# Penguin77jp/RaytracingMin

Measured on AMD Instinct MI355X. Metric: Msamples/s (W*H*spp/s), Cornell box 1080p@1024spp, higher is better.
Workload: dtype f64; 1 GPU; cornellBoxSetting.json rows 0:1080 of 1920x1080 1024spp (SS 4 x S 64), L1 repaired, max_bounces 8, seed 0x5EED, host-libm sin/cos (RTM_MODE_HOST_TRIG), interleaved 8-row bands over 1 GPU(s) + one gather; sample_split_waves_per_tile=8, collective=none (one rank, frame stays in HBM)

## Files before the change

include/rtm_debug.h:

```cpp
#ifndef RTM_DEBUG_H
#define RTM_DEBUG_H

#include "rtm.h"

#ifdef __cplusplus
extern "C" {
#endif

int rtm_debug_math_probe(int op, const double* a, const double* b, size_t n, double* out);
int rtm_debug_trig_table(int entries, double* out);
int rtm_debug_selfcheck(int kind, unsigned long long* mismatches);
int rtm_debug_wf_nearest(int kind, const rtm_sphere* spheres, size_t n, const double* org, const double* dir,
                         size_t n_rays, int32_t* out_id, double* out_t);
int rtm_debug_fp64_peak(int waves_per_simd, double min_ms, double* tflops, double* kernel_ms);
int rtm_debug_grid_nearest(const rtm_sphere* spheres, size_t n, const double* org, const double* dir, size_t n_rays,
                           int32_t* out_id, double* out_t, uint32_t* out_tests, uint32_t* out_steps, uint64_t* info);
int rtm_debug_grid_build(const rtm_sphere* spheres, size_t n, uint64_t* info, double* pads, uint32_t* ranges, size_t ranges_cap,
                         uint32_t* items, size_t items_cap, int32_t* big, size_t big_cap);
int rtm_debug_scene_grid(const rtm_scene* scene, uint64_t* info, uint32_t* ranges, size_t ranges_cap, uint32_t* items,
                         size_t items_cap, int32_t* big, size_t big_cap, uint64_t extra[2]);
int rtm_debug_scene_facts(const rtm_sphere* spheres, size_t n, uint64_t facts[2]);
int rtm_debug_zero_term_facts(const rtm_sphere* spheres, size_t n, uint64_t facts[2]);
int rtm_debug_axis_rows(const rtm_sphere* spheres, size_t n, double* rows);
int rtm_debug_wall_pairs(const rtm_sphere* spheres, size_t n, uint64_t facts[2]);
int rtm_debug_component_bench(int which, const rtm_sphere* spheres, size_t n, int reps, int blocks, int lds_pad,
                              double* cycles_per_rep);
int rtm_debug_denoise_variance_kernel(int form, const rtm_denoise_var_params* params, int32_t width, int32_t height, int device,
                                      const rtm_aov_buffers* guide_dev, void* work_dev, float* variance_out_dev, void* stream);
int rtm_debug_matte_rank(int32_t super_samples, int32_t layers, int device, const int32_t* ids_dev, size_t n_pixels,
                         int32_t* id_out_dev, float* coverage_out_dev, float* alpha_out_dev, void* stream);

#ifdef __cplusplus
}
#endif
#endif
```

raytracingmin_amd/_lib.py:

```python
import ctypes as C
import os

_HERE = os.path.dirname(os.path.abspath(__file__))
LIB_PATH = os.environ.get("RTM_LIB_OVERRIDE") or os.path.join(_HERE, "librtm_hip.so")

RTM_OK = 0
MODE_LITERAL, MODE_REPAIRED = 0, 1
MODE_HOST_TRIG = 0x100
MODE_COUNT_TESTS = 0x200
MODE_SURFACE_SAMPLE = 0x400
MODES = {"literal": MODE_LITERAL, "repaired": MODE_REPAIRED, 0: 0, 1: 1}


class RtmError(RuntimeError):
    def __init__(self, status, what, detail=""):
        self.status = status
        super().__init__(f"{what}: {detail}" if detail else what)


class rtm_camera(C.Structure):
    _fields_ = [("origin", C.c_double * 3), ("target", C.c_double * 3), ("up", C.c_double * 3),
                ("fov", C.c_float), ("_pad", C.c_float)]


# ... 186 lines not shown
    "rtm_read_pfm": (C.c_int, [C.c_char_p, _P(C.c_int), _P(C.c_int), _P(C.c_int), C.c_void_p, C.c_size_t]),
}
DEBUG_SIGNATURES = {
    "rtm_debug_math_probe": (C.c_int, [C.c_int, C.c_void_p, C.c_void_p, C.c_size_t, C.c_void_p]),
    "rtm_debug_selfcheck": (C.c_int, [C.c_int, C.POINTER(C.c_uint64)]),
    "rtm_debug_trig_table": (C.c_int, [C.c_int, C.c_void_p]),
    "rtm_debug_fp64_peak": (C.c_int, [C.c_int, C.c_double, C.POINTER(C.c_double), C.POINTER(C.c_double)]),
    "rtm_debug_wf_nearest": (C.c_int, [C.c_int, C.c_void_p, C.c_size_t, C.c_void_p, C.c_void_p, C.c_size_t,
                                       C.c_void_p, C.c_void_p]),
    "rtm_debug_grid_nearest": (C.c_int, [C.c_void_p, C.c_size_t, C.c_void_p, C.c_void_p, C.c_size_t, C.c_void_p, C.c_void_p,
                                         C.c_void_p, C.c_void_p, C.c_void_p]),
    "rtm_debug_scene_facts": (C.c_int, [C.c_void_p, C.c_size_t, C.c_void_p]),
    "rtm_debug_zero_term_facts": (C.c_int, [C.c_void_p, C.c_size_t, C.c_void_p]),
    "rtm_debug_axis_rows": (C.c_int, [C.c_void_p, C.c_size_t, C.c_void_p]),
    "rtm_debug_wall_pairs": (C.c_int, [C.c_void_p, C.c_size_t, C.c_void_p]),
    "rtm_debug_grid_build": (C.c_int, [C.c_void_p, C.c_size_t, C.c_void_p, C.c_void_p, C.c_void_p, C.c_size_t, C.c_void_p,
                                       C.c_size_t, C.c_void_p, C.c_size_t]),
    "rtm_debug_scene_grid": (C.c_int, [C.c_void_p, C.c_void_p, C.c_void_p, C.c_size_t, C.c_void_p, C.c_size_t, C.c_void_p, C.c_size_t,
                                       C.c_void_p]),
    "rtm_debug_denoise_variance_kernel": (C.c_int, [C.c_int, _P(rtm_denoise_var_params), C.c_int32, C.c_int32, C.c_int,
                                                    _P(rtm_aov_buffers), C.c_void_p, C.c_void_p, C.c_void_p]),
    "rtm_debug_matte_rank": (C.c_int, [C.c_int32, C.c_int32, C.c_int, C.c_void_p, C.c_size_t, C.c_void_p, C.c_void_p, C.c_void_p,
                                       C.c_void_p]),
    "rtm_debug_component_bench": (C.c_int, [C.c_int, C.c_void_p, C.c_size_t, C.c_int, C.c_int, C.c_int,
                                            C.POINTER(C.c_double)]),
}
ABI_VERSION = 5

_lib = None

# ... 33 lines not shown
```

raytracingmin_amd/csrc/rtm_api.cpp:

```cpp
#include <exception>

#include "../../include/rtm_debug.h"
#include "rtm_internal.h"

#define RTM_GUARD(call)                                  \
    try {                                                \
        return (call);                                   \
    } catch (const std::exception& e) {                  \
        rtm::set_last_error(e.what());                   \
        return RTM_ERR_INVALID_ARGUMENT;                 \
    } catch (...) {                                      \
        rtm::set_last_error("unknown exception");        \
        return RTM_ERR_INVALID_ARGUMENT;                 \
    }

extern "C" {

int rtm_abi_version(void) { return RTM_ABI_VERSION; }

const char* rtm_strerror(int status) {
    switch (status) {
        case RTM_OK: return "ok";
        case RTM_ERR_INVALID_ARGUMENT: return "invalid argument";
        case RTM_ERR_INVALID_SCENE: return "invalid scene";
// ... 183 lines not shown
                           int32_t* out_id, double* out_t, uint32_t* out_tests, uint32_t* out_steps, uint64_t* info) {
    RTM_GUARD(rtm::grid_nearest_probe(sp, n, org, dir, n_rays, out_id, out_t, out_tests, out_steps, info))
}
int rtm_debug_grid_build(const rtm_sphere* sp, size_t n, uint64_t* info, double* pads, uint32_t* ranges, size_t ranges_cap,
                         uint32_t* items, size_t items_cap, int32_t* big, size_t big_cap) {
    RTM_GUARD(rtm::grid_build_host(sp, n, info, pads, ranges, ranges_cap, items, items_cap, big, big_cap))
}
int rtm_debug_scene_grid(const rtm_scene* scene, uint64_t* info, uint32_t* ranges, size_t ranges_cap, uint32_t* items,
                         size_t items_cap, int32_t* big, size_t big_cap, uint64_t extra[2]) {
    RTM_GUARD(rtm::scene_grid_probe(scene, info, ranges, ranges_cap, items, items_cap, big, big_cap, extra))
}
int rtm_debug_scene_facts(const rtm_sphere* sp, size_t n, uint64_t facts[2]) { RTM_GUARD(rtm::scene_facts_host(sp, n, facts)) }
int rtm_debug_zero_term_facts(const rtm_sphere* sp, size_t n, uint64_t facts[2]) { RTM_GUARD(rtm::zero_term_facts_host(sp, n, facts)) }
int rtm_debug_axis_rows(const rtm_sphere* sp, size_t n, double* rows) { RTM_GUARD(rtm::axis_rows_host(sp, n, rows)) }
int rtm_debug_wall_pairs(const rtm_sphere* sp, size_t n, uint64_t facts[2]) { RTM_GUARD(rtm::wall_pairs_host(sp, n, facts)) }
int rtm_debug_fp64_peak(int waves_per_simd, double min_ms, double* tflops, double* kernel_ms) {
    RTM_GUARD(rtm::fp64_peak(waves_per_simd, min_ms, tflops, kernel_ms))
}

int rtm_scene_load_json(const char* path, int literal_loader, rtm_settings* settings,
                        rtm_sphere* spheres, size_t capacity, size_t* n_spheres) {
    RTM_GUARD(rtm::scene_load_json(path, literal_loader, settings, spheres, capacity, n_spheres))
}
int rtm_scene_parse_json(const char* text, size_t len, int literal_loader, rtm_settings* settings,
                         rtm_sphere* spheres, size_t capacity, size_t* n_spheres) {
    RTM_GUARD(rtm::scene_parse_json(text, len, literal_loader, settings, spheres, capacity, n_spheres))
}
int rtm_scene_save_sample_json(const char* path) { RTM_GUARD(rtm::scene_save_sample_json(path)) }
int rtm_scene_make_stress(uint64_t seed, size_t n, rtm_settings* settings, rtm_sphere* spheres) {
    RTM_GUARD(rtm::scene_make_stress(seed, n, settings, spheres))
// ... 35 lines not shown
```

raytracingmin_amd/csrc/rtm_device.h:

```cpp
#pragma once
#include <hip/hip_runtime.h>
#include <stdint.h>

#ifndef RTM_NS
#define RTM_NS rtm
#endif
#ifndef RTM_TOL
#define RTM_TOL 0
#endif

namespace RTM_NS {

struct D3 {
    double x, y, z;
};

__device__ __forceinline__ D3 d3(double x, double y, double z) { return D3{x, y, z}; }
__device__ __forceinline__ D3 operator+(D3 a, D3 b) { return D3{a.x + b.x, a.y + b.y, a.z + b.z}; }
__device__ __forceinline__ D3 operator-(D3 a, D3 b) { return D3{a.x - b.x, a.y - b.y, a.z - b.z}; }
__device__ __forceinline__ D3 operator*(D3 a, D3 b) { return D3{a.x * b.x, a.y * b.y, a.z * b.z}; }
__device__ __forceinline__ D3 operator*(D3 a, double s) { return D3{a.x * s, a.y * s, a.z * s}; }
__device__ __forceinline__ D3 operator/(D3 a, double s) { return D3{a.x / s, a.y / s, a.z / s}; }

__device__ __forceinline__ D3 fold_step(const D3 c, const D3 L, const D3 e) {
// ... 182 lines not shown
    const double cosv = c1 + __builtin_fma(t * t, p, c3);
    double s = __builtin_fma(t, k[10], k[11]);
    s = __builtin_fma(t, s, k[12]);
    s = __builtin_fma(t, s, k[13]);
    s = __builtin_fma(t, s, k[14]);
    const double v = hi * t;
    const double sinv = __builtin_fma(v, __builtin_fma(t, s, k[15]), hi);
    const LaneMask odd = lane_mask((q & 1) != 0);
    const int flip = (q & 2) ? (int)0x80000000 : 0;
    const double so = sel_f64(odd, cosv, sinv);
    const double co = sel_f64(odd, -sinv, cosv);
    sn = __hiloint2double(__double2hiint(so) ^ flip, __double2loint(so));
    cs = __hiloint2double(__double2hiint(co) ^ flip, __double2loint(co));
}
constexpr int kTrigTabEntries = 16384;
struct TrigTabWord {
    double s, c;
    int fi;
};
__device__ __forceinline__ TrigTabWord sincos_turn24_tab_load(const double2* __restrict__ tab, const uint32_t m) {
    const uint32_t t = m + 512u;
    unsigned off = (t >> 6) & ((unsigned)(kTrigTabEntries - 1) * (unsigned)sizeof(double2));
    asm volatile("" : "+v"(off));
    const double2 e = *reinterpret_cast<const double2*>(reinterpret_cast<const char*>(tab) + off);
    return TrigTabWord{e.x, e.y, (int)(t & 1023u) - 512};
}
__device__ __forceinline__ void sincos_tab_point_apply(const double ws, const double wc, const double r, double& sn, double& cs) {
    const double t = r * r;
    const double cr = __builtin_fma(t, __builtin_fma(t, 1.0 / 24.0, -0.5), 1.0);
    const double sr = __builtin_fma(r * t, -1.0 / 6.0, r);
// ... 66 lines not shown
```

raytracingmin_amd/csrc/rtm_internal.h:

```cpp
#pragma once
#include <stddef.h>
#include <stdint.h>

#include <string>

#include "../../include/rtm.h"

namespace rtm {

void set_last_error(const std::string& s);
const char* last_error();

int device_count(int* count);
int num_variants();
int output_rows(const rtm_options* opt);
int release_scratch(int device);
int stream_release(int device, void* stream);
int wf_nearest_probe(int kind, const rtm_sphere* sp, size_t n, const double* org, const double* dir, size_t n_rays,
                     int32_t* out_id, double* out_t);
const char* variant_name(int v);
int scene_create(const rtm_sphere* sp, size_t n, int on_device, int device, rtm_scene** out);
int scene_create_device(const rtm_sphere* sp_dev, size_t n, int device, void* stream, rtm_scene** out);
int scene_create_objects(const rtm_object* objs, size_t n, int device, rtm_scene** out);
int intersect_objects_batch(const rtm_object* objs, const double* org, const double* dir, size_t n, int mode,
// ... 66 lines not shown
int selfcheck(int kind, unsigned long long* mismatches);
int grid_nearest_probe(const rtm_sphere* sp, size_t n, const double* org, const double* dir, size_t n_rays, int32_t* out_id,
                       double* out_t, uint32_t* out_tests, uint32_t* out_steps, uint64_t* info);
int scene_facts_host(const rtm_sphere* sp, size_t n, uint64_t* facts);
int zero_term_facts_host(const rtm_sphere* sp, size_t n, uint64_t* facts);
int axis_rows_host(const rtm_sphere* sp, size_t n, double* rows);
int wall_pairs_host(const rtm_sphere* sp, size_t n, uint64_t* facts);
int grid_build_host(const rtm_sphere* sp, size_t n, uint64_t* info, double* pads, uint32_t* ranges, size_t ranges_cap,
                    uint32_t* items, size_t items_cap, int32_t* big, size_t big_cap);
int scene_grid_probe(const rtm_scene* sc, uint64_t* info, uint32_t* ranges, size_t ranges_cap, uint32_t* items, size_t items_cap,
                     int32_t* big, size_t big_cap, uint64_t* extra);
int fp64_peak(int waves_per_simd, double min_ms, double* tflops, double* kernel_ms);
int math_probe(int op, const double* a, const double* b, size_t n, double* out);
int launch_tol(const void* render_params, size_t params_bytes, unsigned grid, size_t lds_pad, void* stream);
int tol_math_probe(int op, const double* a_dev, const double* b_dev, size_t n, double* out_dev);
int trig_table_host(int entries, double* out);
void release_trig_tab(int device);

int scene_parse_json(const char* text, size_t len, int literal_loader, rtm_settings* st,
                     rtm_sphere* spheres, size_t capacity, size_t* n_spheres);
int scene_parse_json_objects(const char* text, size_t len, int literal_loader, rtm_settings* st,
                             rtm_object* objects, size_t capacity, size_t* n_objects);
int scene_load_json_objects(const char* path, int literal_loader, rtm_settings* st, rtm_object* objects,
                            size_t capacity, size_t* n_objects);
int scene_load_json(const char* path, int literal_loader, rtm_settings* st, rtm_sphere* spheres,
                    size_t capacity, size_t* n_spheres);
int scene_save_sample_json(const char* path);
int scene_make_stress(uint64_t seed, size_t n, rtm_settings* st, rtm_sphere* spheres);
int quantise(const double* image, size_t n_values, uint8_t* out);
int write_bmp(const char* filename, int w, int h, int comp, const void* data);
// ... 6 lines not shown
```

raytracingmin_amd/csrc/rtm_kernels.hip:

```cpp
#include <hip/hip_runtime.h>

#include <cfloat>
#include <cmath>
#include <cstdio>
#include <cstdlib>
#include <cstring>
#include <algorithm>
#include <atomic>
#include <thread>
#include <map>
#include <memory>
#include <mutex>
#include <shared_mutex>
#include <tuple>
#include <string>
#include <type_traits>
#include <vector>

#include "../../include/rtm.h"
#include "rtm_device.h"
#include "rtm_host.h"
#include "rtm_path.h"

#include "rtm_render_kernel.h"
// ... 1132 lines not shown
constexpr int deep_lds_levels() { return sizeof(RecT) == 1 ? 64 : 32; }
static bool needs_pool(const RenderParams& P) { return !(P.max_bounces >= 0 && P.max_bounces < 16); }

static size_t debug_lds_pad() {
    static const size_t pad = [] {
        const char* e = std::getenv("RTM_DEBUG_LDS_PAD");
        return e ? (size_t)std::strtoul(e, nullptr, 10) : (size_t)0;
    }();
    return pad;
}

template <class M, unsigned F, typename RecT, int LDS_D, int WPE>
static bool launch_exact_n(const RenderParams& P, unsigned grid, hipStream_t stream) {
    const size_t pad = debug_lds_pad();
    unsigned unit_tab;
    render_lds_bytes<F, RecT, LDS_D>(P.scene.n, pad, &unit_tab);
#define RTM_AXIS_CASE(k, sig)                                                                           \
    if (P.scene.n == k && P.scene.axis_pat == sig && P.mode == RTM_MODE_REPAIRED && unit_tab == 1u) {   \
        launch_tiles<M, F, axis_unroll(k, sig), RecT, LDS_D, WPE>(P, grid, pad, stream);                \
        return true;                                                                                    \
    }
    RTM_AXIS_SIGNATURES(RTM_AXIS_CASE)
#undef RTM_AXIS_CASE
    if constexpr ((F & kPack8) != 0) {
        switch (P.scene.n) {
#define RTM_EXACT_N(k)                                                             \
    case k:                                                                        \
        launch_tiles<M, F, -100 - k, RecT, LDS_D, WPE>(P, grid, pad, stream);      \
        return true;
            RTM_EXACT_N(1) RTM_EXACT_N(2) RTM_EXACT_N(3) RTM_EXACT_N(4) RTM_EXACT_N(5) RTM_EXACT_N(6) RTM_EXACT_N(7)
#undef RTM_EXACT_N
// ... 1617 lines not shown
```

raytracingmin_amd/csrc/rtm_kernels_tol.hip:

```cpp
#define RTM_NS rtm_tol
#define RTM_TOL 1
#include <hip/hip_runtime.h>

#include <cmath>
#include <cstdlib>
#include <cstring>
#include <map>
#include <mutex>
#include <vector>

#include "rtm_internal.h"
#include "rtm_render_kernel.h"

namespace rtm_tol {

static bool compact_launch(const RenderParams& P) {
    const double cam = std::sqrt(P.cam_org.x * P.cam_org.x + P.cam_org.y * P.cam_org.y + P.cam_org.z * P.cam_org.z);
    return (P.scene.fold_flags & kSceneCompact) != 0u && cam <= kCompactExtent;
}
static bool expanded_form_launch(const RenderParams& P) {
    const unsigned e = (P.scene.fold_flags >> kSceneAxisReachShift) & kSceneAxisReachMask;
    const double cam = std::sqrt(P.cam_org.x * P.cam_org.x + P.cam_org.y * P.cam_org.y + P.cam_org.z * P.cam_org.z);
    return e != 0u && cam <= std::ldexp(1.0, (int)e - 128);
}

constexpr unsigned kTolCapped = kLdsTab | kPark | kPack8 | kDefer | kSteal;
constexpr unsigned kTolAny = kLdsTab | kPark | kDefer | kPackL;
constexpr int kTolWavesPerSimd = 4;

template <unsigned F>
static void launch_n(const RenderParams& P, unsigned grid, size_t lds_pad, hipStream_t stream) {
    constexpr int LDS_D = (F & kPackL) != 0 ? 0 : 16;
    unsigned unit_tab;
    render_lds_bytes<F, uint8_t, LDS_D>(P.scene.n, lds_pad, &unit_tab);
    const bool axis = P.mode == RTM_MODE_REPAIRED && unit_tab == 1u && compact_launch(P) && expanded_form_launch(P);
    const unsigned shared_k = (P.scene.fold_flags >> kSceneSharedKShift) & kSceneSharedKMask;
    constexpr bool kPairsShape = (F & (kPackL | kSplit)) != (kPackL | kSplit);
    const unsigned pairs = kPairsShape && (P.scene.fold_flags & kSceneWallPairs) != 0u ? kAxisPairsBit : 0u;
#define RTM_AXIS_CASE(k, sig)                                                                                    \
    if (P.scene.n == k && P.scene.axis_pat == ((sig) & 0xFFFFu) && ((shared_k << kAxisSharedKShift) | pairs) == ((sig) & ~0xFFFFu) && axis) { \
        launch_tiles<MathFast, F, axis_unroll(k, sig), uint8_t, LDS_D, kTolWavesPerSimd>(P, grid, lds_pad, stream); \
        return;                                                                                                  \
    }
    if constexpr (kPairsShape) {
        RTM_AXIS_CASE(7, kAxisSigCornell7Pairs)
    }
    RTM_AXIS_CASE(7, kAxisSigCornell7Walls)
#undef RTM_AXIS_CASE
#define RTM_AXIS_CASE(k, sig)                                                                                    \
// ... 122 lines not shown
namespace rtm {

int trig_table_host(int entries, double* out) {
    if (!out || entries < 1 || entries > (1 << 20)) return RTM_ERR_INVALID_ARGUMENT;
    const long double step = 6.283185307179586476925286766559L / (long double)entries;
    for (int i = 0; i < entries; ++i) {
        const long double a = (long double)i * step;
        out[2 * i] = (double)sinl(a);
        out[2 * i + 1] = (double)cosl(a);
    }
    return RTM_OK;
}

namespace {
std::mutex g_trig_tab_mu;
std::map<int, double2*> g_trig_tab;
}

static int ensure_trig_tab(const double2** out) {
    int device = 0;
    if (hipGetDevice(&device) != hipSuccess) return RTM_ERR_HIP;
    std::lock_guard<std::mutex> lock(g_trig_tab_mu);
    const auto it = g_trig_tab.find(device);
    if (it != g_trig_tab.end()) {
        *out = it->second;
        return RTM_OK;
    }
    constexpr size_t kBytes = (size_t)rtm_tol::kTrigTabEntries * sizeof(double2);
    std::vector<double> host(2 * (size_t)rtm_tol::kTrigTabEntries);
    const int rc = trig_table_host(rtm_tol::kTrigTabEntries, host.data());
    if (rc != RTM_OK) return rc;
    void* dev = nullptr;
    if (hipMalloc(&dev, kBytes) != hipSuccess) {
        (void)hipGetLastError();
        return RTM_ERR_HIP;
    }
    if (hipMemcpy(dev, host.data(), kBytes, hipMemcpyHostToDevice) != hipSuccess || hipStreamSynchronize(nullptr) != hipSuccess) {
        (void)hipGetLastError();
        (void)hipFree(dev);
        return RTM_ERR_HIP;
    }
    g_trig_tab[device] = static_cast<double2*>(dev);
    *out = static_cast<const double2*>(dev);
    return RTM_OK;
}

void release_trig_tab(int device) {
    std::lock_guard<std::mutex> lock(g_trig_tab_mu);
    for (auto it = g_trig_tab.begin(); it != g_trig_tab.end();) {
        if (device < 0 || it->first == device) {
            (void)hipSetDevice(it->first);
            (void)hipDeviceSynchronize();
            (void)hipFree(it->second);
            it = g_trig_tab.erase(it);
        } else {
            ++it;
        }
    }
}

int tol_math_probe(int op, const double* a_dev, const double* b_dev, size_t n, double* out_dev) {
    const double2* tab = nullptr;
    if (op == 42 || op == 43 || op == 46 || op == 47) {
        if (ensure_trig_tab(&tab) != RTM_OK) {
            set_last_error("tolerance row: the sin / cos table could not be allocated on the device");
            return RTM_ERR_HIP;
        }
    }
    rtm_tol::tol_math_probe_kernel<<<(unsigned)((n + 255) / 256), 256>>>(op, a_dev, b_dev, n, out_dev, tab);
    return hipGetLastError() == hipSuccess ? RTM_OK : RTM_ERR_HIP;
}

int launch_tol(const void* params, size_t params_bytes, unsigned grid, size_t lds_pad, void* stream_v) {
    rtm_tol::RenderParams P;
    if (params_bytes != sizeof P) {
        set_last_error("tolerance row: RenderParams layout mismatch between the two translation units");
        return RTM_ERR_INVALID_ARGUMENT;
    }
    std::memcpy(&P, params, sizeof P);
    P.scene.trig_fix = nullptr;
    const double2* trig_tab = nullptr;
    if (ensure_trig_tab(&trig_tab) != RTM_OK) {
        set_last_error("tolerance row: the sin / cos table could not be allocated on the device");
        return RTM_ERR_HIP;
    }
    P.trig_tab = trig_tab;
    hipStream_t stream = (hipStream_t)stream_v;
    const bool any_depth = P.max_bounces < 0 || P.max_bounces > 8;
    if ((!any_depth && P.steal_ws == nullptr) || P.scene.n < 1 || P.scene.n > 24 || P.scene.plane != nullptr ||
        P.sample_end >= 65536u) {
        set_last_error("variant 18 (fp64 tolerance row) serves all-sphere scenes of 1..24 spheres with fewer than 65 536 samples per pixel");
        return RTM_ERR_UNSUPPORTED;
    }
    if (P.prim_masks == nullptr) {
        set_last_error("tolerance row: no primary-ray mask buffer");
        return RTM_ERR_INVALID_ARGUMENT;
    }
    const unsigned n_tiles_all = P.split > 1 ? P.split_first + P.n_tiles : grid;
    static const bool no_masks = [] {
        const char* e = std::getenv("RTM_DEBUG_TOL_PRIMFIX");
        return e && e[0] == '0';
// ... 18 lines not shown
```

raytracingmin_amd/csrc/rtm_path.h:

```cpp
#pragma once
#include <cfloat>
#include <type_traits>

#include "../../include/rtm.h"
#include "rtm_device.h"

namespace RTM_NS {


__device__ __forceinline__ double seq_rcp(const double y) {
    double r = __builtin_amdgcn_rcp(y);
    double e = __builtin_fma(-y, r, 1.0);
#if RTM_TOL
    return __builtin_fma(r, __builtin_fma(e, e, e), r);
#else
    r = __builtin_fma(r, e, r);
    e = __builtin_fma(-y, r, 1.0);
    return __builtin_fma(r, e, r);
#endif
}
__device__ __forceinline__ double seq_quot(const double x, const double y, const double r) {
#if RTM_TOL
    (void)y;
    return x * r;
// ... 545 lines not shown
        const double* g = lgeom + id * 4;
        return D3{g[0], g[1], g[2]};
    }
    __device__ __forceinline__ double kd(int id) const { return lmat[id * 8 + 6]; }
    __device__ __forceinline__ double kd24(int id) const { return lmat[id * 8 + 7]; }
    __device__ __forceinline__ D3 emission(int id) const {
        const double* m = lmat + id * 8;
        return D3{m[3], m[4], m[5]};
    }
    __device__ __forceinline__ D3 color_kd(int id) const {
        const double* m = lmat + id * 8;
        return D3{m[0], m[1], m[2]};
    }
};

struct SceneLdsObjects {
    SceneView v;
    const double* lgeom;
    const double* lmat;
    const double* lnrm;
    static constexpr bool kHasNormTable = false;
    static constexpr bool kPlanes = true;
    static constexpr bool kNeverPlanes = false;
    __device__ __forceinline__ int n() const { return v.n; }
    __device__ __forceinline__ double4 geom_uniform(int i) const { return load_geom_uniform(v.geom, i); }
    __device__ __forceinline__ D3 center(int id) const {
        const double* g = lgeom + id * 4;
        return D3{g[0], g[1], g[2]};
    }
    __device__ __forceinline__ bool is_plane(int id) const { return __double2hiint(lgeom[id * 4 + 3]) < 0; }
// ... 204 lines not shown
        b = py * dir.y - A.Pxz;
        D4 = b * b - (py * py + A.Qxz) + g.w;
    } else if (pat == 3u) {
        const double pz = g.z - org.z;
        b = pz * dir.z - A.Pxy;
        D4 = b * b - (A.Qxy + pz * pz) + g.w;
    } else {
        const D3 p_o = d3(g.x - org.x, g.y - org.y, g.z - org.z);
        b = dot(p_o, dir);
        D4 = b * b - dot(p_o, p_o) + g.w;
    }
}
__device__ __forceinline__ double pair_signed_origin(const unsigned pat, const D3 org, const D3 dir) {
    const double oa = pat == 1u ? org.x : pat == 2u ? org.y : org.z;
    const double da = pat == 1u ? dir.x : pat == 2u ? dir.y : dir.z;
    const uint32_t sign = (uint32_t)__double2hiint(da) & 0x80000000u;
    return __hiloint2double((int)((uint32_t)__double2hiint(oa) ^ sign), __double2loint(oa));
}
__device__ __forceinline__ bool pair_unproven(const AxisRow r, const unsigned pat, const double ooK, const D3 org, const D3 dir,
                                              const AxisShared& A) {
    const double da = pat == 1u ? dir.x : pat == 2u ? dir.y : dir.z;
    double bu;
#if defined(__HIP_DEVICE_COMPILE__)
    asm("v_fma_f64 %0, -%1, |%2|, -%3" : "=v"(bu) : "s"(r.c), "v"(da), "v"(A.od));
#else
    bu = __builtin_fma(-r.c, __builtin_fabs(da), -A.od);
#endif
    const double qu = __builtin_fma(-r.m2c, pair_signed_origin(pat, org, dir), ooK);
    return !(bu <= -kPairBeta && __builtin_fma(-2.0 * kPairTau, bu, qu) >= 0.0);
}
__device__ __forceinline__ void pair_disc(const AxisRow r, const unsigned pat, const double ooK, const D3 org, const D3 dir,
                                          const AxisShared& A, double& b, double& D4) {
// ... 997 lines not shown
```

raytracingmin_amd/csrc/rtm_render_kernel.h:

```cpp
#pragma once
#include <type_traits>

#include "rtm_path.h"

namespace RTM_NS {

struct RenderParams {
    SceneView scene;
    int W, H, S, SS;
    int row_begin, row_end;
    int band_count, band_index;
    int tiles_x;
    int mode, max_bounces;
    unsigned total_samples;
    unsigned sample_begin, sample_end, seeded;
    double preview_scale;
    float rate;
    double dSS, dS;
    double inv_ss, inv_s;
    D3 cam_org, ax, by, cz;
    uint64_t seed_mult;
    double* __restrict__ out64;
    float* __restrict__ out32;
    uint8_t* __restrict__ out8;
// ... 4 lines not shown
    unsigned long long* __restrict__ stamps;
    unsigned n_tiles, split, split_head, split_len, split_first;
    double* __restrict__ partial;
    unsigned char* __restrict__ contrib;
    unsigned* __restrict__ split_counts;
    unsigned char* __restrict__ steal_ws;
    unsigned steal_rows, steal_depth;
    unsigned magic_S, magic_SS;
    unsigned xcd_on, xcd_q, xcd_rem;
    unsigned unit_tab;
    const unsigned long long* __restrict__ prim_masks;
    const double* __restrict__ prim_dirs;
    unsigned* __restrict__ nz_bits;
    const unsigned* __restrict__ tile_map;
    unsigned frame_tiles;
    const double2* __restrict__ trig_tab;
};
constexpr size_t kTermRowBytes = 3 * 64 * sizeof(double) + 64 * sizeof(unsigned short);
constexpr size_t kStealRowBytes = 3 * 64 * sizeof(double) + 64 * sizeof(unsigned);
constexpr size_t kStealHdrBytes = 256;
__host__ __device__ inline size_t steal_tile_bytes(unsigned rows) { return kStealHdrBytes + 3 * 64 * sizeof(double) + (size_t)rows * kStealRowBytes; }

__device__ __forceinline__ unsigned long long stamp_now() {
    unsigned long long t;
    __builtin_amdgcn_sched_barrier(0);
    asm volatile("s_memtime %0\n s_waitcnt lgkmcnt(0)" : "=s"(t)::"memory");
    __builtin_amdgcn_sched_barrier(0);
    return t;
}

constexpr int kPoolLevels = 960;
// ... 26 lines not shown
        }
    }
    __device__ __forceinline__ int pop(int d) {
        if (d < LDS_D) return (int)lds[d * 64 + lane];
        if (slot < 0 || d - LDS_D >= kPoolLevels) return 0;
        return (int)(reinterpret_cast<const RecT*>(P->pool) + (size_t)slot * kPoolLevels)[d - LDS_D];
    }
    static constexpr int kCapacity = LDS_D + kPoolLevels;
};

constexpr size_t kUnitTableBytes = (size_t)(kShadeConstCount - kTrigConstCount) * sizeof(double);
inline bool unit_table_fits(size_t lds) {
    auto waves = [](size_t b) { const size_t w = b ? (size_t)163840 / b : 16; return w > 16 ? (size_t)16 : w; };
    return waves(lds) == waves(lds + kUnitTableBytes);
}
__host__ __device__ inline size_t lds_table_bytes(int n) { return ((size_t)n * 7 + ((size_t)n + 1) * 8) * sizeof(double); }

__device__ __forceinline__ D3 primary_dir(const RenderParams& P, int x, int y, int sx, int sy) {
    const double px = 2.0 * ((double)x + (double)(P.rate * (float)sx)) / P.W - 1.0;
    const double py = 2.0 * ((double)y + (double)(P.rate * (float)sy)) / P.H - 1.0;
    return normalize((P.ax * px + P.by * py) + P.cz);
}

__device__ __forceinline__ D3 primary_dir_lds(const RenderParams& P, const double* cam, int x, int y, int sx,
                                              int sy) {
#if RTM_TOL
#pragma clang fp contract(off)
    const double px = 2.0 * ((double)x + (double)(P.rate * (float)sx)) / P.W - 1.0;
    const double py = 2.0 * ((double)y + (double)(P.rate * (float)sy)) / P.H - 1.0;
    const double vx = (cam[0] * px + cam[3] * py) + cam[6];
    const double vy = (cam[1] * px + cam[4] * py) + cam[7];
// ... 74 lines not shown
    int hi = (int)((reversed << ((unsigned)hit_id & 63u)) >> 32);
    asm("" : "+v"(hi));
    return hi < 0;
}

constexpr unsigned kLdsTab = 1u << 0, kPark = 1u << 1, kStamp = 1u << 2, kPack8 = 1u << 3, kSplit = 1u << 4;
constexpr unsigned kDefer = 1u << 5, kPackL = 1u << 6, kReuse = 1u << 7, kPlanes = 1u << 8, kSteal = 1u << 9;

constexpr int kFoldRing = 128;
constexpr size_t kFoldQueueBytes = kFoldRing * 16 + 3 * 64 * 8 + 64 * 8 + 64 * 4;
constexpr size_t kFoldQueueBytesS = kFoldRing * 16 + 64 * 4 + 64 * 4;
constexpr size_t kFoldQueueBytesLS = kFoldQueueBytesS + kFoldRing * 8 + 64 * 8;


template <unsigned F, typename RecT, int LDS_D>
inline size_t render_lds_bytes(int n, size_t pad, unsigned* unit_tab) {
    size_t b = (F & kLdsTab) ? lds_table_bytes(n) : 0;
    b += (10 + kTrigConstCount) * sizeof(double);
    if (F & kPark) b += 6 * 64 * sizeof(double);
    if (!(F & (kPack8 | kPackL))) b += (size_t)LDS_D * 64 * sizeof(RecT);
    if (F & kDefer) b += (F & kReuse) ? kFoldQueueBytes : (F & kPackL) ? kFoldQueueBytesLS : kFoldQueueBytesS;
    if (F & kSteal) b += 2 * 64 * sizeof(unsigned) + (RTM_TOL ? 64 * sizeof(unsigned long long) : 0);
    b += pad;
    *unit_tab = unit_table_fits(b) ? 1u : 0u;
    return b + (*unit_tab ? kUnitTableBytes : 0);
}

template <class M, unsigned F, int UNROLL, typename RecT, int LDS_D, int WPE>
__global__ __launch_bounds__(64, WPE) void render_tiles_kernel(const RenderParams P) {
    constexpr bool LDS_TAB = (F & kLdsTab) != 0, PARK = (F & kPark) != 0, STAMP = (F & kStamp) != 0;
    constexpr bool PACK8 = (F & kPack8) != 0, SPLIT = (F & kSplit) != 0, DEFER = (F & kDefer) != 0;
    constexpr bool PACKL = (F & kPackL) != 0, REUSE = (F & kReuse) != 0, PLANES = (F & kPlanes) != 0;
    constexpr bool STEAL = (F & kSteal) != 0;
    static_assert(!STEAL || (DEFER && PACK8 && !REUSE && !PACKL), "sample stealing rides on the deferred fold with packed records");
    static_assert(!PLANES || (LDS_TAB && !REUSE), "plane scenes ride on the LDS tables");
    static_assert(!SPLIT || DEFER, "the sample split's small waves store their terms from the fold queue");
    static_assert(!DEFER || ((PACK8 || PACKL) && PARK && !STAMP), "the fold queue rides on packed records and the LDS accumulator");
    static_assert(!REUSE || (DEFER && PACK8 && !SPLIT), "primary-hit reuse rides on the deferred fold with packed records");
    static_assert(!PACKL || (DEFER && !PACK8 && LDS_D == 0 && sizeof(RecT) == 1), "PACKL: deferred fold, byte records, pooled stack only");
    extern __shared__ __attribute__((aligned(16))) unsigned char lds_raw[];
    const int lane = threadIdx.x;
    const unsigned block_tile = (SPLIT && blockIdx.x >= P.split_first) ? P.split_first + (blockIdx.x - P.split_first) % P.n_tiles
                                                                        : blockIdx.x;
    const unsigned block_frame_tile = frame_tile(P, block_tile);
    if (block_frame_tile == ~0u) return;
    const int scene_n = P.scene.n;
    double* lgeom = reinterpret_cast<double*>(lds_raw);
    double* lmat = lgeom + (LDS_TAB ? scene_n * 4 : 0);
    double* lnrm = lmat + (LDS_TAB ? (scene_n + 1) * 8 : 0);
    double* cam = reinterpret_cast<double*>(lds_raw + (LDS_TAB ? lds_table_bytes(scene_n) : 0));
    double* trig = cam + 10;
    const bool unit_tab = UNROLL <= -1000 ? true : (P.unit_tab != 0u);
    double* park = trig + (unit_tab ? kShadeConstCount : kTrigConstCount);
#if RTM_TOL
    ShadeLds shade_lds_tab(trig, unit_tab);
    shade_lds_tab.tab = P.trig_tab;
    const ShadeLds shade_lds = shade_lds_tab;
#else
    const ShadeLds shade_lds(trig, unit_tab);
#endif
    RecT* rec = reinterpret_cast<RecT*>(park + (PARK ? 6 * 64 : 0));
    constexpr bool kScatter = DEFER && (PACK8 || PACKL) && !REUSE;
    uint4* fq_in = reinterpret_cast<uint4*>(park + 6 * 64);
    double* fq_out = reinterpret_cast<double*>(fq_in + kFoldRing);
    unsigned long long* fq_fifo = kScatter ? reinterpret_cast<unsigned long long*>(fq_in + kFoldRing)
                                           : reinterpret_cast<unsigned long long*>(fq_out + 3 * 64);
    unsigned* fq_pend = kScatter ? reinterpret_cast<unsigned*>(fq_fifo) + 64 : reinterpret_cast<unsigned*>(fq_fifo + 64);
    unsigned long long* fq_in1 = reinterpret_cast<unsigned long long*>(fq_pend + 64);
    unsigned long long* rec_w1 = fq_in1 + kFoldRing;
    unsigned short* fq_tag = reinterpret_cast<unsigned short*>(fq_fifo);
    static_assert(kFoldRing * sizeof(unsigned short) <= 64 * sizeof(unsigned), "the tags fit the FIFO array, and the counts' that takes its place");
// ... 5 lines not shown
    if (lane < 9) {
        const double v9[9] = {P.ax.x, P.ax.y, P.ax.z, P.by.x, P.by.y, P.by.z, P.cz.x, P.cz.y, P.cz.z};
        double pick = v9[0];
#pragma unroll
        for (int k = 1; k < 9; ++k) pick = (lane == k) ? v9[k] : pick;
        cam[lane] = pick;
    }
    {
        const unsigned first = block_tile * (unsigned)(P.SS * P.SS);
        const double slot = __longlong_as_double((long long)(((unsigned long long)block_frame_tile << 32) | first));
        if (lane == 9) cam[9] = slot;
    }
    __syncthreads();
    if constexpr (LDS_TAB) {
        const double* gsrc = reinterpret_cast<const double*>(P.scene.geom);
        for (int i = lane; i < scene_n * 4; i += 64) lgeom[i] = gsrc[i];
        for (int i = lane; i < (scene_n + 1) * 8; i += 64) lmat[i] = P.scene.mat[i];
        for (int i = lane; i < scene_n; i += 64) {
            if (PLANES && gsrc[i * 4 + 3] < 0.0) {
                lnrm[i * 3] = P.scene.plane[(size_t)i * 16 + 3];
                lnrm[i * 3 + 1] = P.scene.plane[(size_t)i * 16 + 4];
                lnrm[i * 3 + 2] = P.scene.plane[(size_t)i * 16 + 5];
                continue;
            }
            fill_norm_row(lnrm + i * 3, gsrc[i * 4 + 3]);
        }
        __syncthreads();
    }
    using Scene = typename std::conditional<PLANES, SceneLdsObjects,
                                            typename std::conditional<LDS_TAB, SceneLds, SceneGlobal>::type>::type;
    Scene sc;
    sc.v = P.scene;
    sc.v.n = scene_n;
    const int mode = UNROLL <= -1000 ? (int)RTM_MODE_REPAIRED : P.mode;
    if constexpr (LDS_TAB) {
        sc.lgeom = lgeom;
        sc.lmat = lmat;
        sc.lnrm = lnrm;
    }

    auto pixel_xy = [&](int& px, int& py) {
        int l = lane;
        asm volatile("" : "+v"(l));
        const unsigned tile = (unsigned)__builtin_amdgcn_readfirstlane((int)reinterpret_cast<const unsigned*>(cam + 9)[1]);
        const int tx = tile % P.tiles_x, ty = tile / P.tiles_x;
        px = tx * 8 + (l & 7);
        py = band_row(P, ty, l >> 3);
    };
    int x, y;
    pixel_xy(x, y);
// ... 801 lines not shown
        __syncthreads();
        if (valid) {
            for (unsigned s = end_own; s < total; ++s) {
                const unsigned e = idx[(s - floor_s) * 64u + (unsigned)lane];
                if (e >= n_terms) continue;
                const double* v = reinterpret_cast<const double*>(rows + (size_t)(e >> 6) * kStealRowBytes) + (e & 63u);
                acc = acc + d3(v[0], v[64], v[128]);
            }
        }
    }
    store_pixel(P, valid, px, py, acc);
}

template <class M, unsigned F, int UNROLL, typename RecT, int LDS_D, int WPE>
void launch_tiles(RenderParams P, unsigned grid, size_t pad, hipStream_t stream) {
    const size_t lds = render_lds_bytes<F, RecT, LDS_D>(P.scene.n, pad, &P.unit_tab);
    render_tiles_kernel<M, F, UNROLL, RecT, LDS_D, WPE><<<grid, 64, lds, stream>>>(P);
}
inline void launch_split_finalize(const RenderParams& P, hipStream_t stream) {
    split_finalize_kernel<<<P.n_tiles, 256, (size_t)P.split_len * (64 * 3 * sizeof(double) + 2 * sizeof(unsigned)), stream>>>(P);
}
inline void launch_steal_finalize(const RenderParams& P, unsigned grid, hipStream_t stream) {
    const unsigned n_whole = P.split > 1 ? P.split_first : grid;
    if (n_whole) steal_finalize_kernel<<<n_whole, 64, (size_t)P.steal_depth * 64 * sizeof(unsigned short), stream>>>(P);
}

__global__ __launch_bounds__(64) void prim_prepass_kernel(const RenderParams P, unsigned long long* __restrict__ masks,
                                                          double* __restrict__ dirs) {
    const int lane = threadIdx.x;
    const unsigned tile = blockIdx.x;
    const unsigned ftile = frame_tile(P, tile);
// ... 34 lines not shown
```

Before: 24210 Msamples/s.

## Pack sphere geometry, normals and kd into 8-double LDS rows; move trig table to device global

For the tolerance kernel path, each sphere's center, radius, normalisation terms and kd are interleaved into one 8-double LDS row, so a hit's per-object data comes from one contiguous row instead of three separate tables. The sin/cos table becomes a __device__ global symbol, which removes a pointer from the kernel parameters. The sign-flip in pair_signed_origin now uses a single bitop3 instruction. The row layout costs one extra double per object in LDS, and the table is no longer freed on release.

New measurement: 24650 Msamples/s (median of 6 runs). 1.8% higher.

```diff
diff --git a/include/rtm_debug.h b/include/rtm_debug.h
--- a/include/rtm_debug.h
+++ b/include/rtm_debug.h
@@ -23,6 +23,7 @@
 int rtm_debug_zero_term_facts(const rtm_sphere* spheres, size_t n, uint64_t facts[2]);
 int rtm_debug_axis_rows(const rtm_sphere* spheres, size_t n, double* rows);
 int rtm_debug_wall_pairs(const rtm_sphere* spheres, size_t n, uint64_t facts[2]);
+int rtm_debug_tol_lds_bytes(int n, int any_depth, int split, int rows, uint64_t out[2]);
 int rtm_debug_component_bench(int which, const rtm_sphere* spheres, size_t n, int reps, int blocks, int lds_pad,
                               double* cycles_per_rep);
 int rtm_debug_denoise_variance_kernel(int form, const rtm_denoise_var_params* params, int32_t width, int32_t height, int device,
diff --git a/raytracingmin_amd/_lib.py b/raytracingmin_amd/_lib.py
--- a/raytracingmin_amd/_lib.py
+++ b/raytracingmin_amd/_lib.py
@@ -224,6 +224,7 @@
     "rtm_debug_zero_term_facts": (C.c_int, [C.c_void_p, C.c_size_t, C.c_void_p]),
     "rtm_debug_axis_rows": (C.c_int, [C.c_void_p, C.c_size_t, C.c_void_p]),
     "rtm_debug_wall_pairs": (C.c_int, [C.c_void_p, C.c_size_t, C.c_void_p]),
+    "rtm_debug_tol_lds_bytes": (C.c_int, [C.c_int, C.c_int, C.c_int, C.c_int, C.c_void_p]),
     "rtm_debug_grid_build": (C.c_int, [C.c_void_p, C.c_size_t, C.c_void_p, C.c_void_p, C.c_void_p, C.c_size_t, C.c_void_p,
                                        C.c_size_t, C.c_void_p, C.c_size_t]),
     "rtm_debug_scene_grid": (C.c_int, [C.c_void_p, C.c_void_p, C.c_void_p, C.c_size_t, C.c_void_p, C.c_size_t, C.c_void_p, C.c_size_t,
diff --git a/raytracingmin_amd/csrc/rtm_api.cpp b/raytracingmin_amd/csrc/rtm_api.cpp
--- a/raytracingmin_amd/csrc/rtm_api.cpp
+++ b/raytracingmin_amd/csrc/rtm_api.cpp
@@ -221,6 +221,7 @@
 int rtm_debug_zero_term_facts(const rtm_sphere* sp, size_t n, uint64_t facts[2]) { RTM_GUARD(rtm::zero_term_facts_host(sp, n, facts)) }
 int rtm_debug_axis_rows(const rtm_sphere* sp, size_t n, double* rows) { RTM_GUARD(rtm::axis_rows_host(sp, n, rows)) }
 int rtm_debug_wall_pairs(const rtm_sphere* sp, size_t n, uint64_t facts[2]) { RTM_GUARD(rtm::wall_pairs_host(sp, n, facts)) }
+int rtm_debug_tol_lds_bytes(int n, int any_depth, int split, int rows, uint64_t out[2]) { RTM_GUARD(rtm::tol_lds_bytes(n, any_depth, split, rows, out)) }
 int rtm_debug_fp64_peak(int waves_per_simd, double min_ms, double* tflops, double* kernel_ms) {
     RTM_GUARD(rtm::fp64_peak(waves_per_simd, min_ms, tflops, kernel_ms))
 }
diff --git a/raytracingmin_amd/csrc/rtm_device.h b/raytracingmin_amd/csrc/rtm_device.h
--- a/raytracingmin_amd/csrc/rtm_device.h
+++ b/raytracingmin_amd/csrc/rtm_device.h
@@ -220,6 +220,7 @@
     cs = __hiloint2double(__double2hiint(co) ^ flip, __double2loint(co));
 }
 constexpr int kTrigTabEntries = 16384;
+__device__ double2 g_trig_tab[kTrigTabEntries];
 struct TrigTabWord {
     double s, c;
     int fi;
diff --git a/raytracingmin_amd/csrc/rtm_internal.h b/raytracingmin_amd/csrc/rtm_internal.h
--- a/raytracingmin_amd/csrc/rtm_internal.h
+++ b/raytracingmin_amd/csrc/rtm_internal.h
@@ -104,6 +104,7 @@
 int math_probe(int op, const double* a, const double* b, size_t n, double* out);
 int launch_tol(const void* render_params, size_t params_bytes, unsigned grid, size_t lds_pad, void* stream);
 int tol_math_probe(int op, const double* a_dev, const double* b_dev, size_t n, double* out_dev);
+int tol_lds_bytes(int n, int any_depth, int split, int rows, uint64_t* out);
 int trig_table_host(int entries, double* out);
 void release_trig_tab(int device);
 
diff --git a/raytracingmin_amd/csrc/rtm_kernels.hip b/raytracingmin_amd/csrc/rtm_kernels.hip
--- a/raytracingmin_amd/csrc/rtm_kernels.hip
+++ b/raytracingmin_amd/csrc/rtm_kernels.hip
@@ -1170,7 +1170,7 @@
 static bool launch_exact_n(const RenderParams& P, unsigned grid, hipStream_t stream) {
     const size_t pad = debug_lds_pad();
     unsigned unit_tab;
-    render_lds_bytes<F, RecT, LDS_D>(P.scene.n, pad, &unit_tab);
+    render_lds_bytes<F, RecT, LDS_D>(P.scene.n, lds_rows_for(-1000), pad, &unit_tab);
 #define RTM_AXIS_CASE(k, sig)                                                                           \
     if (P.scene.n == k && P.scene.axis_pat == sig && P.mode == RTM_MODE_REPAIRED && unit_tab == 1u) {   \
         launch_tiles<M, F, axis_unroll(k, sig), RecT, LDS_D, WPE>(P, grid, pad, stream);                \
diff --git a/raytracingmin_amd/csrc/rtm_kernels_tol.hip b/raytracingmin_amd/csrc/rtm_kernels_tol.hip
--- a/raytracingmin_amd/csrc/rtm_kernels_tol.hip
+++ b/raytracingmin_amd/csrc/rtm_kernels_tol.hip
@@ -32,7 +32,7 @@
 static void launch_n(const RenderParams& P, unsigned grid, size_t lds_pad, hipStream_t stream) {
     constexpr int LDS_D = (F & kPackL) != 0 ? 0 : 16;
     unsigned unit_tab;
-    render_lds_bytes<F, uint8_t, LDS_D>(P.scene.n, lds_pad, &unit_tab);
+    render_lds_bytes<F, uint8_t, LDS_D>(P.scene.n, lds_rows_for(-1000), lds_pad, &unit_tab);
     const bool axis = P.mode == RTM_MODE_REPAIRED && unit_tab == 1u && compact_launch(P) && expanded_form_launch(P);
     const unsigned shared_k = (P.scene.fold_flags >> kSceneSharedKShift) & kSceneSharedKMask;
     constexpr bool kPairsShape = (F & (kPackL | kSplit)) != (kPackL | kSplit);
@@ -185,15 +185,15 @@
 
 namespace {
 std::mutex g_trig_tab_mu;
-std::map<int, double2*> g_trig_tab;
+std::map<int, const double2*> g_trig_tab_filled;
 }
 
 static int ensure_trig_tab(const double2** out) {
     int device = 0;
     if (hipGetDevice(&device) != hipSuccess) return RTM_ERR_HIP;
     std::lock_guard<std::mutex> lock(g_trig_tab_mu);
-    const auto it = g_trig_tab.find(device);
-    if (it != g_trig_tab.end()) {
+    const auto it = g_trig_tab_filled.find(device);
+    if (it != g_trig_tab_filled.end()) {
         *out = it->second;
         return RTM_OK;
     }
@@ -202,39 +202,36 @@
     const int rc = trig_table_host(rtm_tol::kTrigTabEntries, host.data());
     if (rc != RTM_OK) return rc;
     void* dev = nullptr;
-    if (hipMalloc(&dev, kBytes) != hipSuccess) {
+    if (hipGetSymbolAddress(&dev, HIP_SYMBOL(rtm_tol::g_trig_tab)) != hipSuccess || dev == nullptr ||
+        hipMemcpy(dev, host.data(), kBytes, hipMemcpyHostToDevice) != hipSuccess || hipStreamSynchronize(nullptr) != hipSuccess) {
         (void)hipGetLastError();
         return RTM_ERR_HIP;
     }
-    if (hipMemcpy(dev, host.data(), kBytes, hipMemcpyHostToDevice) != hipSuccess || hipStreamSynchronize(nullptr) != hipSuccess) {
-        (void)hipGetLastError();
-        (void)hipFree(dev);
-        return RTM_ERR_HIP;
-    }
-    g_trig_tab[device] = static_cast<double2*>(dev);
+    g_trig_tab_filled[device] = static_cast<const double2*>(dev);
     *out = static_cast<const double2*>(dev);
     return RTM_OK;
 }
 
-void release_trig_tab(int device) {
-    std::lock_guard<std::mutex> lock(g_trig_tab_mu);
-    for (auto it = g_trig_tab.begin(); it != g_trig_tab.end();) {
-        if (device < 0 || it->first == device) {
-            (void)hipSetDevice(it->first);
-            (void)hipDeviceSynchronize();
-            (void)hipFree(it->second);
-            it = g_trig_tab.erase(it);
-        } else {
-            ++it;
-        }
-    }
+void release_trig_tab(int device) { (void)device; }
+
+int tol_lds_bytes(int n, int any_depth, int split, int rows, uint64_t* out) {
+    using namespace rtm_tol;
+    if (!out || n < 1 || n > 24) return RTM_ERR_INVALID_ARGUMENT;
+    unsigned unit = 0u;
+    const bool r = rows != 0;
+    size_t b;
+    if (any_depth) b = split ? render_lds_bytes<kTolAny | kSplit, uint8_t, 0>(n, r, 0, &unit) : render_lds_bytes<kTolAny, uint8_t, 0>(n, r, 0, &unit);
+    else b = split ? render_lds_bytes<kTolCapped | kSplit, uint8_t, 16>(n, r, 0, &unit) : render_lds_bytes<kTolCapped, uint8_t, 16>(n, r, 0, &unit);
+    out[0] = (uint64_t)b;
+    out[1] = unit;
+    return RTM_OK;
 }
 
 int tol_math_probe(int op, const double* a_dev, const double* b_dev, size_t n, double* out_dev) {
     const double2* tab = nullptr;
     if (op == 42 || op == 43 || op == 46 || op == 47) {
         if (ensure_trig_tab(&tab) != RTM_OK) {
-            set_last_error("tolerance row: the sin / cos table could not be allocated on the device");
+            set_last_error("tolerance row: the sin / cos table could not be written on the device");
             return RTM_ERR_HIP;
         }
     }
@@ -252,10 +249,9 @@
     P.scene.trig_fix = nullptr;
     const double2* trig_tab = nullptr;
     if (ensure_trig_tab(&trig_tab) != RTM_OK) {
-        set_last_error("tolerance row: the sin / cos table could not be allocated on the device");
+        set_last_error("tolerance row: the sin / cos table could not be written on the device");
         return RTM_ERR_HIP;
     }
-    P.trig_tab = trig_tab;
     hipStream_t stream = (hipStream_t)stream_v;
     const bool any_depth = P.max_bounces < 0 || P.max_bounces > 8;
     if ((!any_depth && P.steal_ws == nullptr) || P.scene.n < 1 || P.scene.n > 24 || P.scene.plane != nullptr ||
diff --git a/raytracingmin_amd/csrc/rtm_path.h b/raytracingmin_amd/csrc/rtm_path.h
--- a/raytracingmin_amd/csrc/rtm_path.h
+++ b/raytracingmin_amd/csrc/rtm_path.h
@@ -583,6 +583,35 @@
     }
 };
 
+constexpr int kLdsRowDoubles = 8;
+struct SceneLdsRows {
+    SceneView v;
+    const double* lrow;
+    const double* lmat;
+    static constexpr bool kHasNormTable = true;
+    static constexpr bool kPlanes = false;
+    static constexpr bool kNeverPlanes = true;
+    __device__ __forceinline__ double norm_m(int id) const { return lrow[id * kLdsRowDoubles + 4]; }
+    __device__ __forceinline__ double norm_rinv(int id) const { return lrow[id * kLdsRowDoubles + 5]; }
+    __device__ __forceinline__ float norm_r2f(int id) const { return reinterpret_cast<const float*>(lrow + id * kLdsRowDoubles + 6)[0]; }
+    __device__ __forceinline__ int n() const { return v.n; }
+    __device__ __forceinline__ double4 geom_uniform(int i) const { return load_geom_uniform(v.geom, i); }
+    __device__ __forceinline__ D3 center(int id) const {
+        const double* g = lrow + id * kLdsRowDoubles;
+        return D3{g[0], g[1], g[2]};
+    }
+    __device__ __forceinline__ double kd(int id) const { return lmat[id * 8 + 6]; }
+    __device__ __forceinline__ double kd24(int id) const { return lrow[id * kLdsRowDoubles + 7]; }
+    __device__ __forceinline__ D3 emission(int id) const {
+        const double* m = lmat + id * 8;
+        return D3{m[3], m[4], m[5]};
+    }
+    __device__ __forceinline__ D3 color_kd(int id) const {
+        const double* m = lmat + id * 8;
+        return D3{m[0], m[1], m[2]};
+    }
+};
+
 struct SceneLdsObjects {
     SceneView v;
     const double* lgeom;
@@ -817,8 +846,12 @@
 __device__ __forceinline__ double pair_signed_origin(const unsigned pat, const D3 org, const D3 dir) {
     const double oa = pat == 1u ? org.x : pat == 2u ? org.y : org.z;
     const double da = pat == 1u ? dir.x : pat == 2u ? dir.y : dir.z;
-    const uint32_t sign = (uint32_t)__double2hiint(da) & 0x80000000u;
-    return __hiloint2double((int)((uint32_t)__double2hiint(oa) ^ sign), __double2loint(oa));
+#if defined(__HIP_DEVICE_COMPILE__)
+    const uint32_t hi = __builtin_amdgcn_bitop3_b32((uint32_t)__double2hiint(oa), (uint32_t)__double2hiint(da), 0x80000000u, 0x78);
+#else
+    const uint32_t hi = (uint32_t)__double2hiint(oa) ^ ((uint32_t)__double2hiint(da) & 0x80000000u);
+#endif
+    return __hiloint2double((int)hi, __double2loint(oa));
 }
 __device__ __forceinline__ bool pair_unproven(const AxisRow r, const unsigned pat, const double ooK, const D3 org, const D3 dir,
                                               const AxisShared& A) {
diff --git a/raytracingmin_amd/csrc/rtm_render_kernel.h b/raytracingmin_amd/csrc/rtm_render_kernel.h
--- a/raytracingmin_amd/csrc/rtm_render_kernel.h
+++ b/raytracingmin_amd/csrc/rtm_render_kernel.h
@@ -42,7 +42,6 @@
     unsigned* __restrict__ nz_bits;
     const unsigned* __restrict__ tile_map;
     unsigned frame_tiles;
-    const double2* __restrict__ trig_tab;
 };
 constexpr size_t kTermRowBytes = 3 * 64 * sizeof(double) + 64 * sizeof(unsigned short);
 constexpr size_t kStealRowBytes = 3 * 64 * sizeof(double) + 64 * sizeof(unsigned);
@@ -99,7 +98,10 @@
     auto waves = [](size_t b) { const size_t w = b ? (size_t)163840 / b : 16; return w > 16 ? (size_t)16 : w; };
     return waves(lds) == waves(lds + kUnitTableBytes);
 }
-__host__ __device__ inline size_t lds_table_bytes(int n) { return ((size_t)n * 7 + ((size_t)n + 1) * 8) * sizeof(double); }
+__host__ __device__ inline size_t lds_table_bytes(int n, bool rows) {
+    return ((size_t)n * (rows ? 8 : 7) + ((size_t)n + 1) * 8) * sizeof(double);
+}
+constexpr bool lds_rows_for(int unroll) { return RTM_TOL != 0 && unroll <= -1000; }
 
 __device__ __forceinline__ D3 primary_dir(const RenderParams& P, int x, int y, int sx, int sy) {
     const double px = 2.0 * ((double)x + (double)(P.rate * (float)sx)) / P.W - 1.0;
@@ -204,8 +206,8 @@
 
 
 template <unsigned F, typename RecT, int LDS_D>
-inline size_t render_lds_bytes(int n, size_t pad, unsigned* unit_tab) {
-    size_t b = (F & kLdsTab) ? lds_table_bytes(n) : 0;
+inline size_t render_lds_bytes(int n, bool rows, size_t pad, unsigned* unit_tab) {
+    size_t b = (F & kLdsTab) ? lds_table_bytes(n, rows) : 0;
     b += (10 + kTrigConstCount) * sizeof(double);
     if (F & kPark) b += 6 * 64 * sizeof(double);
     if (!(F & (kPack8 | kPackL))) b += (size_t)LDS_D * 64 * sizeof(RecT);
@@ -235,16 +237,18 @@
     const unsigned block_frame_tile = frame_tile(P, block_tile);
     if (block_frame_tile == ~0u) return;
     const int scene_n = P.scene.n;
+    constexpr bool kRowTab = LDS_TAB && lds_rows_for(UNROLL);
+    static_assert(!(kRowTab && PLANES), "a plane's normal has no place in a sphere's row");
     double* lgeom = reinterpret_cast<double*>(lds_raw);
-    double* lmat = lgeom + (LDS_TAB ? scene_n * 4 : 0);
-    double* lnrm = lmat + (LDS_TAB ? (scene_n + 1) * 8 : 0);
-    double* cam = reinterpret_cast<double*>(lds_raw + (LDS_TAB ? lds_table_bytes(scene_n) : 0));
+    double* lmat = lgeom + (LDS_TAB ? scene_n * (kRowTab ? kLdsRowDoubles : 4) : 0);
+    [[maybe_unused]] double* lnrm = lmat + (LDS_TAB ? (scene_n + 1) * 8 : 0);
+    double* cam = reinterpret_cast<double*>(lds_raw + (LDS_TAB ? lds_table_bytes(scene_n, kRowTab) : 0));
     double* trig = cam + 10;
     const bool unit_tab = UNROLL <= -1000 ? true : (P.unit_tab != 0u);
     double* park = trig + (unit_tab ? kShadeConstCount : kTrigConstCount);
 #if RTM_TOL
     ShadeLds shade_lds_tab(trig, unit_tab);
-    shade_lds_tab.tab = P.trig_tab;
+    shade_lds_tab.tab = g_trig_tab;
     const ShadeLds shade_lds = shade_lds_tab;
 #else
     const ShadeLds shade_lds(trig, unit_tab);
@@ -280,9 +284,14 @@
     __syncthreads();
     if constexpr (LDS_TAB) {
         const double* gsrc = reinterpret_cast<const double*>(P.scene.geom);
-        for (int i = lane; i < scene_n * 4; i += 64) lgeom[i] = gsrc[i];
+        for (int i = lane; i < scene_n * 4; i += 64) lgeom[kRowTab ? (i >> 2) * kLdsRowDoubles + (i & 3) : i] = gsrc[i];
         for (int i = lane; i < (scene_n + 1) * 8; i += 64) lmat[i] = P.scene.mat[i];
         for (int i = lane; i < scene_n; i += 64) {
+            if constexpr (kRowTab) {
+                fill_norm_row(lgeom + i * kLdsRowDoubles + 4, gsrc[i * 4 + 3]);
+                lgeom[i * kLdsRowDoubles + 7] = P.scene.mat[i * 8 + 7];
+                continue;
+            }
             if (PLANES && gsrc[i * 4 + 3] < 0.0) {
                 lnrm[i * 3] = P.scene.plane[(size_t)i * 16 + 3];
                 lnrm[i * 3 + 1] = P.scene.plane[(size_t)i * 16 + 4];
@@ -293,13 +302,17 @@
         }
         __syncthreads();
     }
+    using SceneTab = typename std::conditional<kRowTab, SceneLdsRows, SceneLds>::type;
     using Scene = typename std::conditional<PLANES, SceneLdsObjects,
-                                            typename std::conditional<LDS_TAB, SceneLds, SceneGlobal>::type>::type;
+                                            typename std::conditional<LDS_TAB, SceneTab, SceneGlobal>::type>::type;
     Scene sc;
     sc.v = P.scene;
     sc.v.n = scene_n;
     const int mode = UNROLL <= -1000 ? (int)RTM_MODE_REPAIRED : P.mode;
-    if constexpr (LDS_TAB) {
+    if constexpr (kRowTab) {
+        sc.lrow = lgeom;
+        sc.lmat = lmat;
+    } else if constexpr (LDS_TAB) {
         sc.lgeom = lgeom;
         sc.lmat = lmat;
         sc.lnrm = lnrm;
@@ -1131,7 +1144,7 @@
 
 template <class M, unsigned F, int UNROLL, typename RecT, int LDS_D, int WPE>
 void launch_tiles(RenderParams P, unsigned grid, size_t pad, hipStream_t stream) {
-    const size_t lds = render_lds_bytes<F, RecT, LDS_D>(P.scene.n, pad, &P.unit_tab);
+    const size_t lds = render_lds_bytes<F, RecT, LDS_D>(P.scene.n, lds_rows_for(UNROLL), pad, &P.unit_tab);
     render_tiles_kernel<M, F, UNROLL, RecT, LDS_D, WPE><<<grid, 64, lds, stream>>>(P);
 }
 inline void launch_split_finalize(const RenderParams& P, hipStream_t stream) {
```
